# ChristophReich1996/Semantic_Pyramid_for_Image_Generation

Hardware: AMD Instinct MI355X
Metric: images/sec full G+D train step, 256x256, bs/GPU=20 (higher is better)
Workload: dtype bf16

## Files before the change

include/sempyr.h:

```cpp
#ifndef SEMPYR_H
#define SEMPYR_H
#include <stdint.h>

#ifdef __cplusplus
extern "C" {
#endif

#define SP_VERSION 1

typedef void* sp_stream_t;

enum sp_status { SP_OK = 0, SP_ERR_INVALID = -1, SP_ERR_LAUNCH = -2, SP_ERR_UNSUPPORTED = -3 };
enum sp_dtype { SP_F32 = 0, SP_BF16 = 1, SP_F8 = 2 ,
                SP_F16 = 3 ,
                SP_F8_F16 = 4  };
enum sp_act { SP_ACT_NONE = 0, SP_ACT_LRELU = 1, SP_ACT_RELU = 2, SP_ACT_TANH = 3 };

int sp_version(void);

enum { SP_TUNE_CONV_TALL = 0, SP_TUNE_IGEMM_DMA = 1, SP_TUNE_WGRAD_ROWS = 2, SP_TUNE_DETERMINISTIC = 3,
       SP_TUNE_SPLITK_TARGET = 4, SP_TUNE_SPLITK_MINSTEPS = 5, SP_TUNE_CONV1X1_DIRECT = 6, SP_TUNE_CONV_SHORT = 7,
       SP_TUNE_WGRAD9_BLOCKS = 8, SP_TUNE_WGRAD_BLOCKS = 9, SP_TUNE_WGRAD_MINSTEPS = 10, SP_TUNE_WGRAD_SMALL_M = 11,
       SP_TUNE_WGRAD_K1_TILE64 = 12, SP_TUNE_WGRAD_ROWS_THIN = 13, SP_TUNE_WGRAD_ROWS_BLOCKS = 14, SP_TUNE_WGRAD_ROWS_SLABS = 15,
       SP_TUNE_CONV_STAGGER = 16, SP_TUNE_CONV1X1_SPLITK = 17, SP_TUNE_WGRAD1X1 = 18, SP_TUNE_CONV_CIN8 = 19, SP_TUNE_CONV_THINCO = 20, SP_TUNE_CONV_PP = 21, SP_TUNE_CONV_PP_PRIO = 22, SP_TUNE_WGRAD_PP = 23, SP_TUNE_BN_ITERS = 24, SP_TUNE_IGEMM_TILE = 25, SP_TUNE_CONV_PPW = 26, SP_TUNE_LINEAR_KS = 27, SP_TUNE_CONV_PP_SPLIT = 28, SP_TUNE_COUNT = 29 };
int sp_set_tuning(int32_t key, int32_t value);
const char* sp_last_error_string(void);
const char* sp_last_route(void);

typedef struct sp_conv_params {
    const void* x;
    const void* w;
    const float* bias;
    void* y;
    const void* res1;
    const void* res2;
    const void* mask_src;
    float mask_neg_slope;
    int32_t n, h, w_, cin_p, cout, ldy, ksize, act, dtype;
    void* workspace;
    int64_t workspace_bytes;
    int32_t pool2;
    int32_t in_up2;
    const float* x_scale;
    const float* w_scale;
    void* y8;
    const float* y8_inv_scale;
    float* y8_amax;
    const float* img_scale;
    int32_t img_split;
    int32_t reserved_;
    int64_t split_pix_;
    const void* tail_w;
    const float* tail_bias;
    void* tail_y;
    int32_t tail_cout, tail_act, tail_ld, reserved2_;
    uint32_t* pool_idx;
    int32_t* split_sync;
} sp_conv_params;
#define SP_CONV_SPLIT_SYNC_BYTES 8192
int sp_conv2d_igemm(const sp_conv_params* p, sp_stream_t stream);
int sp_conv2d_workspace(int32_t n, int32_t h, int32_t w_, int32_t cin_p, int32_t cout, int32_t ksize, int32_t dtype,
                        int64_t* bytes_out);

int sp_conv2d_wgrad(const void* x, const void* dy, float* dw, int32_t n, int32_t h, int32_t w_,
                    int32_t cin_p, int32_t cout, int32_t ld_dy, int32_t ksize, int32_t dtype,
                    sp_stream_t stream);

int sp_conv2d_wgrad_fused(const void* x, const void* dy, float* dw, float* dbias, const void* w_packed, float* dot,
                          float* workspace, int64_t workspace_floats, int32_t n, int32_t h, int32_t w_, int32_t cin_p,
                          int32_t cout, int32_t ld_dy, int32_t ksize, int32_t dtype, sp_stream_t stream);
int sp_conv2d_wgrad_accum(const void* x, const void* dy, float* dw, float* dbias, float* workspace, int64_t workspace_floats,
                          int32_t n, int32_t h, int32_t w_, int32_t cin_p, int32_t cout, int32_t ld_dy, int32_t ksize,
                          int32_t dtype, sp_stream_t stream);
int sp_conv2d_wgrad_accum_pooled(const void* x, const void* dy, float* dw, float* dbias, float* workspace, int64_t workspace_floats,
                                 int32_t n, int32_t h, int32_t w_, int32_t cin_p, int32_t cout, int32_t ld_dy, int32_t ksize,
                                 int32_t dtype, sp_stream_t stream);
int sp_conv2d_wgrad_workspace(int32_t n, int32_t h, int32_t w_, int32_t cin_p, int32_t cout, int32_t ksize,
// ... 224 lines not shown
```

semantic_pyramid_for_image_generation_amd/_lib.py:

```python
from __future__ import annotations

import ctypes
import os
import re
from typing import Dict, List, Tuple

_HERE = os.path.dirname(os.path.abspath(__file__))
HEADER = os.path.join(os.path.dirname(_HERE), "include", "sempyr.h")
LIB_PATH = os.environ.get("SEMPYR_LIB") or os.path.join(_HERE, "libsempyr.so")

SP_F32, SP_BF16, SP_F8, SP_F16, SP_F8_F16 = 0, 1, 2, 3, 4
ACT_NONE, ACT_LRELU, ACT_RELU, ACT_TANH = 0, 1, 2, 3

TUNE_KEYS = {"SP_CONV_TALL": 0, "SP_IGEMM_DMA": 1, "SP_WGRAD_ROWS": 2, "SP_DETERMINISTIC": 3, "SP_SPLITK_TARGET": 4,
             "SP_SPLITK_MINSTEPS": 5, "SP_CONV1X1_DIRECT": 6, "SP_CONV_SHORT": 7, "SP_WGRAD9_BLOCKS": 8, "SP_WGRAD_BLOCKS": 9,
             "SP_WGRAD_MINSTEPS": 10, "SP_WGRAD_SMALL_M": 11, "SP_WGRAD_K1_TILE64": 12, "SP_WGRAD_ROWS_THIN": 13,
             "SP_WGRAD_ROWS_BLOCKS": 14, "SP_WGRAD_ROWS_SLABS": 15, "SP_CONV_STAGGER": 16, "SP_CONV1X1_SPLITK": 17, "SP_WGRAD1X1": 18, "SP_CONV_CIN8": 19, "SP_CONV_THINCO": 20,
             "SP_CONV_PP": 21, "SP_CONV_PP_PRIO": 22, "SP_WGRAD_PP": 23, "SP_BN_ITERS": 24, "SP_IGEMM_TILE": 25, "SP_CONV_PPW": 26, "SP_LINEAR_KS": 27, "SP_CONV_PP_SPLIT": 28}


SP_CONV_SPLIT_SYNC_BYTES = 8192


class SpConvParams(ctypes.Structure):
    _fields_ = [("x", ctypes.c_void_p), ("w", ctypes.c_void_p), ("bias", ctypes.c_void_p), ("y", ctypes.c_void_p),
                ("res1", ctypes.c_void_p), ("res2", ctypes.c_void_p), ("mask_src", ctypes.c_void_p),
                ("mask_neg_slope", ctypes.c_float),
                ("n", ctypes.c_int32), ("h", ctypes.c_int32), ("w_", ctypes.c_int32), ("cin_p", ctypes.c_int32),
                ("cout", ctypes.c_int32), ("ldy", ctypes.c_int32), ("ksize", ctypes.c_int32), ("act", ctypes.c_int32),
                ("dtype", ctypes.c_int32), ("workspace", ctypes.c_void_p), ("workspace_bytes", ctypes.c_int64),
                ("pool2", ctypes.c_int32), ("in_up2", ctypes.c_int32),
                ("x_scale", ctypes.c_void_p), ("w_scale", ctypes.c_void_p), ("y8", ctypes.c_void_p),
                ("y8_inv_scale", ctypes.c_void_p), ("y8_amax", ctypes.c_void_p),
                ("img_scale", ctypes.c_void_p), ("img_split", ctypes.c_int32), ("reserved_", ctypes.c_int32),
                ("split_pix_", ctypes.c_int64),
                ("tail_w", ctypes.c_void_p), ("tail_bias", ctypes.c_void_p), ("tail_y", ctypes.c_void_p),
                ("tail_cout", ctypes.c_int32), ("tail_act", ctypes.c_int32), ("tail_ld", ctypes.c_int32), ("reserved2_", ctypes.c_int32),
                ("pool_idx", ctypes.c_void_p), ("split_sync", ctypes.c_void_p)]


class SpConvGeneralParams(ctypes.Structure):
    _fields_ = [("struct_bytes", ctypes.c_int32), ("dtype", ctypes.c_int32),
                ("x", ctypes.c_void_p), ("w", ctypes.c_void_p), ("bias", ctypes.c_void_p), ("y", ctypes.c_void_p),
                ("n", ctypes.c_int32), ("h", ctypes.c_int32), ("w_", ctypes.c_int32), ("cin_p", ctypes.c_int32),
                ("ldx", ctypes.c_int32), ("cout", ctypes.c_int32), ("ldy", ctypes.c_int32), ("kh", ctypes.c_int32),
                ("kw", ctypes.c_int32), ("stride_h", ctypes.c_int32), ("stride_w", ctypes.c_int32), ("pad_h", ctypes.c_int32),
                ("pad_w", ctypes.c_int32), ("act", ctypes.c_int32)]

    def __init__(self, **kw):
        super().__init__(struct_bytes=ctypes.sizeof(SpConvGeneralParams), **kw)


class SpSnLayer(ctypes.Structure):
    _fields_ = [("w", ctypes.c_void_p), ("u", ctypes.c_void_p), ("v", ctypes.c_void_p),
                ("scratch_off", ctypes.c_int64), ("part_off", ctypes.c_int64), ("fwd_off", ctypes.c_int64),
                ("dgrad_off", ctypes.c_int64),
                ("rows", ctypes.c_int32), ("cols", ctypes.c_int32), ("cin", ctypes.c_int32), ("taps", ctypes.c_int32),
                ("cin_p", ctypes.c_int32), ("cout_p", ctypes.c_int32), ("kind", ctypes.c_int32),
                ("pack_block0", ctypes.c_int32)]


class SpSnBwdLayer(ctypes.Structure):
    _fields_ = [("w", ctypes.c_void_p), ("dw_off", ctypes.c_int64), ("dot_off", ctypes.c_int64),
                ("scratch_off", ctypes.c_int64), ("grad_off", ctypes.c_int64),
                ("rows", ctypes.c_int32), ("cols", ctypes.c_int32), ("cin", ctypes.c_int32), ("taps", ctypes.c_int32),
                ("cin_p", ctypes.c_int32), ("plain", ctypes.c_int32), ("db_off", ctypes.c_int32),
                ("bias_off", ctypes.c_int32)]


class SpRecLevel(ctypes.Structure):
    _fields_ = [("real", ctypes.c_void_p), ("fake", ctypes.c_void_p), ("mask", ctypes.c_void_p), ("dfake", ctypes.c_void_p),
# ... 60 lines not shown
```

semantic_pyramid_for_image_generation_amd/csrc/common.h:

```cpp
#pragma once
#include <hip/hip_runtime.h>
#include <stdint.h>
#include "../../include/sempyr.h"

typedef __attribute__((ext_vector_type(4))) float f32x4_t;
typedef __attribute__((ext_vector_type(4))) short s16x4_t;
typedef float sp_f32x2_t __attribute__((ext_vector_type(2)));

struct bf16 { uint16_t v; };
#ifdef SP_H16_FP16
typedef __attribute__((ext_vector_type(8))) _Float16 bf16x8_t;
typedef _Float16 sp_h16x2_t __attribute__((ext_vector_type(2)));
#define __builtin_amdgcn_mfma_f32_16x16x32_bf16 __builtin_amdgcn_mfma_f32_16x16x32_f16
#define SP_H16_ONE_PAIR 0x3C003C00u
__device__ __forceinline__ float bf16_bits_to_f32(uint32_t h) { return (float)__builtin_bit_cast(_Float16, (uint16_t)h); }
__device__ __forceinline__ uint32_t f32x2_to_bf16x2(float lo, float hi) {
    const sp_f32x2_t f = {lo, hi};
    return __builtin_bit_cast(uint32_t, __builtin_convertvector(f, sp_h16x2_t));
}
__device__ __forceinline__ float h16_lo_to_f32(uint32_t w) { return (float)__builtin_bit_cast(_Float16, (uint16_t)(w & 0xffffu)); }
__device__ __forceinline__ float h16_hi_to_f32(uint32_t w) { return (float)__builtin_bit_cast(_Float16, (uint16_t)(w >> 16)); }
#else
typedef __attribute__((ext_vector_type(8))) __bf16 bf16x8_t;
typedef __bf16 sp_bf16x2_t __attribute__((ext_vector_type(2)));
// ... 76 lines not shown
            asm("v_max_f32 %0, %1, %2" : "=v"(v[r]) : "v"(v[r]), "v"(s));
        }
    } else if (act == SP_ACT_RELU) {
#pragma unroll
        for (int r = 0; r < N; ++r) v[r] = fmaxf(v[r], 0.f);
    } else if (TANH_OK && act == SP_ACT_TANH) {
#pragma unroll
        for (int r = 0; r < N; ++r) v[r] = tanhf(v[r]);
    }
}

extern "C" void sp_set_error(const char* fmt, ...);
extern "C" void sp_note_route(const char* name);
#define SP_CHECK_ARG(cond, ...) do { if (!(cond)) { sp_set_error(__VA_ARGS__); return SP_ERR_INVALID; } } while (0)
#define SP_LAUNCH_CHECK() do { hipError_t e_ = hipGetLastError(); if (e_ != hipSuccess) { \
    sp_set_error("%s:%d HIP launch failed: %s", __FILE__, __LINE__, hipGetErrorString(e_)); return SP_ERR_LAUNCH; } } while (0)

static inline int sp_div_up(long a, long b) { return (int)((a + b - 1) / b); }

template <typename T, int V> struct VecIO;
template <> struct VecIO<float, 4> {
    static __device__ __forceinline__ void ld(const float* p, float (&o)[4]) { Elem<float>::ld4(p, o); }
    static __device__ __forceinline__ void st(float* p, const float (&o)[4]) { Elem<float>::st4(p, o); }
};
template <> struct VecIO<bf16, 4> {
    static __device__ __forceinline__ void ld(const bf16* p, float (&o)[4]) { Elem<bf16>::ld4(p, o); }
    static __device__ __forceinline__ void st(bf16* p, const float (&o)[4]) { Elem<bf16>::st4(p, o); }
};
template <> struct VecIO<bf16, 8> {
    static __device__ __forceinline__ void ld(const bf16* p, float (&o)[8]) {
        const uint4 v = *reinterpret_cast<const uint4*>(p);
        o[0] = bf16_bits_to_f32(v.x & 0xffffu); o[1] = bf16_bits_to_f32(v.x >> 16);
        o[2] = bf16_bits_to_f32(v.y & 0xffffu); o[3] = bf16_bits_to_f32(v.y >> 16);
        o[4] = bf16_bits_to_f32(v.z & 0xffffu); o[5] = bf16_bits_to_f32(v.z >> 16);
        o[6] = bf16_bits_to_f32(v.w & 0xffffu); o[7] = bf16_bits_to_f32(v.w >> 16);
    }
    static __device__ __forceinline__ void st(bf16* p, const float (&o)[8]) {
        uint4 v;
        v.x = f32x2_to_bf16x2(o[0], o[1]);
        v.y = f32x2_to_bf16x2(o[2], o[3]);
        v.z = f32x2_to_bf16x2(o[4], o[5]);
        v.w = f32x2_to_bf16x2(o[6], o[7]);
        *reinterpret_cast<uint4*>(p) = v;
    }
};

extern int* const sp_g_tune;
static inline int sp_tune(int key, int dflt) { return sp_g_tune[key] >= 0 ? sp_g_tune[key] : dflt; }
static inline bool sp_deterministic(int dtype) { return sp_g_tune[SP_TUNE_DETERMINISTIC] >= 0 ? sp_g_tune[SP_TUNE_DETERMINISTIC] != 0 : dtype == SP_F32; }
int sp_conv_pp_launch(const sp_conv_params& p, int th, hipStream_t s);
long sp_conv_pp_split_workspace(int n, int h, int w, int cin_p, int cout);
long sp_conv_pp_split_workspace_w16(int n, int h, int cin_p, int cout);
long sp_conv_pp_rounds100(long total, int cin_p, long workspace_bytes);
int sp_conv_ppw_launch(const sp_conv_params& p, hipStream_t s);
long sp_conv_ppw_split_workspace(int n, int h, int w, int cin_p, int cout);
long sp_conv_ppw_rounds100(long total, int cin_p, long workspace_bytes);
int sp_conv_ppw_covers(const sp_conv_params& p);
bool spq_push_reduce(const float* slabs, int nsplit, long n_dw, float* dw, const float* bias_slabs, int bias_ld, int cout, float* dbias);
int sp_wgrad_rows_launch(const void* x, const void* dy, float* dw, float* dbias, int n, int h, int w, int cin, int cout,
                         int ld_dy, float* ws, long ws_floats, int dy_up2, hipStream_t s);
long sp_wgrad_rows_workspace(int n, int h, int w, int cin, int cout);
int sp_wgrad_rows_launch_pair(const void* x, const void* dy, float* dw_a, float* dbias_a, float* dw_b, float* dbias_b, int n, int split,
                              int h, int w, int cin, int cout, int ld_dy, float* ws, long ws_floats, int dy_up2, hipStream_t s);
int sp_wgrad1x1_launch(const void* x, const void* dy, float* dw, float* dbias, int n, int h, int w, int cin, int cout, int ld_dy,
                       float* ws, long ws_floats, hipStream_t s);
long sp_wgrad1x1_workspace(int n, int h, int w, int cin, int cout, int ld_dy);
int sp_wgrad1x1_launch_pair(const void* x, const void* dy, float* dw_a, float* dbias_a, float* dw_b, float* dbias_b, int n, int split, int h, int w,
                            int cin, int cout, int ld_dy, float* ws, long ws_floats, hipStream_t s);
int sp_wgrad3x3_cin8_launch_pair(const void* x, const void* dy, float* dw_a, float* dbias_a, float* dw_b, float* dbias_b, int n, int split, int h,
                                 int w, int cout, int ld_dy, float* ws, long ws_floats, hipStream_t s);
int sp_wgrad3x3_cin8_launch(const void* x, const void* dy, float* dw, float* dbias, int n, int h, int w, int cout, int ld_dy, float* ws,
                            long ws_floats, hipStream_t s);
long sp_wgrad3x3_cin8_workspace(int n, int h, int w, int cout, int ld_dy);
```

semantic_pyramid_for_image_generation_amd/csrc/conv_igemm.hip:

```cpp
#include "conv_common.h"

namespace {

template <typename T, int WCO, int WPX, int FCO, int FPX>
__global__ __launch_bounds__(256) void conv_igemm_kernel(sp_conv_params p) {
    constexpr int CO_T = WCO * FCO * 16, PX_T = WPX * FPX * 16;
    constexpr int E = 16 / (int)sizeof(T);
    constexpr int KC = 8 * E;
    constexpr int W_CH = CO_T * 8, X_CH = PX_T * 8;
    constexpr int W_PER = (W_CH + 255) / 256, X_PER = (X_CH + 255) / 256;
    constexpr int STAGE = (CO_T + PX_T) * 128;
    extern __shared__ __attribute__((aligned(16))) char smem[];

    const int tid = threadIdx.x, lane = tid & 63, wave = tid >> 6;
    const int wco = wave / WPX, wpx = wave % WPX;
    const int H = p.h, W = p.w_, CIN = p.cin_p;
    const long M = (long)p.n * H * W;
    const long px0 = (long)blockIdx.x * PX_T;
    const int co0 = blockIdx.y * CO_T;
    const int taps = p.ksize * p.ksize;
    const int kchunks = (CIN + KC - 1) / KC;
    const int nk = taps * kchunks;
    const T* __restrict__ xg = reinterpret_cast<const T*>(p.x);
    const T* __restrict__ wg = reinterpret_cast<const T*>(p.w);
// ... 1322 lines not shown

template <int KC>
int launch_thinco(const sp_conv_params& p, hipStream_t s) {
    constexpr int LDS = TN_HH * TN_HW * (KC * 64 + 16);
    static bool attr_set = false;
    if (!attr_set) {
        hipError_t e = hipFuncSetAttribute(reinterpret_cast<const void*>(conv3x3_thinco_kernel<KC>), hipFuncAttributeMaxDynamicSharedMemorySize, LDS);
        if (e != hipSuccess) { sp_set_error("hipFuncSetAttribute(LDS=%d) failed: %s", LDS, hipGetErrorString(e)); return SP_ERR_LAUNCH; }
        attr_set = true;
    }
    const long blocks = (long)p.n * (p.h / TN_TH) * (p.w_ / TN_TW);
    sp_note_route("conv3x3_thinco");
    hipLaunchKernelGGL(conv3x3_thinco_kernel<KC>, dim3((unsigned)blocks), dim3(256), LDS, s, p);
    SP_LAUNCH_CHECK();
    return SP_OK;
}

template <typename T>
int dispatch(const sp_conv_params& p, hipStream_t s) {
    const long M = (long)p.n * p.h * p.w_;
    if (sizeof(T) == 2 && p.ksize == 3 && p.cout <= 4 && (p.cin_p == 32 || p.cin_p == 64) && !p.pool2 && !p.in_up2 && p.h % TN_TH == 0 &&
        p.w_ % TN_TW == 0 && sp_tune(SP_TUNE_CONV_THINCO, 1) && sp_tune(SP_TUNE_CONV_TALL, 1) <= 1)
        return p.cin_p == 64 ? launch_thinco<2>(p, s) : launch_thinco<1>(p, s);
    if (sizeof(T) == 2 && p.ksize == 3 && p.cin_p == 8 && p.cout % 16 == 0 && p.cout <= 64 && (p.ldy & 7) == 0 && !p.pool2 && !p.in_up2 &&
        p.h % C8_TH == 0 && p.w_ % C8_TW == 0 && sp_tune(SP_TUNE_CONV_CIN8, 1) && sp_tune(SP_TUNE_CONV_TALL, 1) <= 1)
        return launch_cin8(p, s);
    if (sizeof(T) == 2 && p.ksize == 1 && p.cin_p > 1024 && ((M + 31) / 32) * ((p.cout + 63) / 64) <= sp_tune(SP_TUNE_CONV1X1_SPLITK, 320))
        return launch_1x1_splitk(p, s);
    if (sizeof(T) == 2 && p.ksize == 1 && p.cin_p <= 1024) {
        const int ks = (p.cin_p + 31) / 32;
        const long blocks = ((M + 31) / 32) * ((p.cout + 63) / 64);
        if (ks >= 4 && ks <= 24 && blocks <= sp_tune(SP_TUNE_CONV1X1_SPLITK, 320)) return launch_1x1_splitk(p, s);
        if (sp_tune(SP_TUNE_CONV1X1_DIRECT, 1)) return launch_1x1_direct(p, s);
    }
    if (p.pool_idx != nullptr) {
        const long esz = p.dtype == SP_F32 ? 4 : 2;
        const bool fits30 = (long)p.n * p.h * p.w_ * p.cin_p * esz < (1L << 30) && (long)p.cout * 9 * p.cin_p * esz < (1L << 30);
        if (p.cout <= 64 && p.h % TL_TH != 0) return launch_halo<T, 64, 1, true>(p, s);
        if (!fits30) { sp_set_error("sp_conv2d_igemm: pool_idx needs operands below 1 GiB (n*h*w*cin_p, cout*9*cin_p)"); return SP_ERR_UNSUPPORTED; }
        if (sizeof(T) == 2 && sp_tune(SP_TUNE_CONV_PP, 1)) {
            const int rc = sp_conv_pp_launch(p, p.cout <= 64 ? 16 : 8, s);
            if (rc != 1) return rc;
        }
        return p.cout <= 64 ? launch_tall<T, 1, 16, true>(p, s) : launch_tall<T, 2, 8, true>(p, s);
    }
    const bool thin_big = p.cout <= 16 && p.cin_p >= 32 && M >= (1L << 18);
    if (p.ksize == 3 && (p.cout > 32 || thin_big) && p.h % HALO_TH == 0 && p.w_ % HALO_TW == 0) {
        const int tall_mode = sp_tune(SP_TUNE_CONV_TALL, 1);
        const long esz = p.dtype == SP_F32 ? 4 : 2;
        const bool fits30 = (long)p.n * p.h * p.w_ * p.cin_p * esz < (1L << 30) && (long)p.cout * 9 * p.cin_p * esz < (1L << 30);
        const bool tall_ok = tall_mode && fits30 && p.h % TL_TH == 0 && p.w_ % TL_TW == 0;
        if (p.cout <= 64) {
            if (tall_ok && sizeof(T) == 2 && p.cout > 16 && tall_mode <= 1 && sp_tune(SP_TUNE_CONV_PP, 1) && !(sp_tune(SP_TUNE_CONV_PP, 1) & 32)) {
                const int rc = sp_conv_pp_launch(p, 16, s);
                if (rc != 1) return rc;
            }
            if (tall_ok) return launch_tall<T, 1>(p, s);
            return launch_halo<T, 64, 1>(p, s);
        }
        const int pp_mode = sizeof(T) == 2 ? sp_tune(SP_TUNE_CONV_PP, 1) : 0;
        if (pp_mode && fits30 && tall_mode <= 1) {
            const long bt = (long)p.n * (p.h / TL_TH) * (p.w_ / TL_TW) * ((p.cout + 127) / 128);
            const long rt = (bt + 255) / 256, rh = (2 * bt + 255) / 256;
            int th = (tall_ok && 19 * rt < 10 * rh) ? 16 : 8;
            if (pp_mode == 8 || (pp_mode == 16 && tall_ok)) th = pp_mode;
            const int ppw_mode = sp_tune(SP_TUNE_CONV_PPW, 1);
            if (tall_ok && ppw_mode && pp_mode == 1 && sp_conv_ppw_covers(p)) {
                const int kch = (p.cin_p + 31) / 32;
                const long ratio = kch >= 12 ? 172 : kch >= 6 ? 185 : kch >= 3 ? 194 : 204;
                const long wsb = (p.workspace != nullptr && p.split_sync != nullptr) ? p.workspace_bytes : 0;
                const long rh100 = sp_conv_pp_rounds100(2 * bt, p.cin_p, wsb);
                const long rt100 = ppw_mode == 3 ? sp_conv_ppw_rounds100(bt, p.cin_p, wsb) : 100 * rt;
                if (ppw_mode == 2 || ratio * rt100 < 100 * rh100) {
                    const int rc = sp_conv_ppw_launch(p, s);
                    if (rc != 1) return rc;
                }
                th = 8;
            }
            if (!(pp_mode == 1 && th == 16)) {
                const int rc = sp_conv_pp_launch(p, th, s);
                if (rc != 1) return rc;
            }
        }
        if (tall_ok) {
            const long bt = (long)p.n * (p.h / TL_TH) * (p.w_ / TL_TW) * ((p.cout + 127) / 128);
            const long rt = (bt + 255) / 256, rh = (2 * bt + 255) / 256;
            if (tall_mode == 2 || 19 * rt < 10 * rh) return launch_tall<T, 2>(p, s);
        }
        const int short_env = sp_tune(SP_TUNE_CONV_SHORT, 1);
        if (fits30 && (tall_mode == 3 || (tall_mode == 1 && short_env))) return launch_tall<T, 2, 8>(p, s);
        return launch_halo<T, 128, 3>(p, s);
    }
    if (sizeof(T) == 2 && p.ksize == 3 && p.w_ == 16 && p.cout > 64) {
        const int ppm = sp_tune(SP_TUNE_CONV_PP, 1);
        if (ppm == 1 || ppm == 3) {
            const int rc = sp_conv_pp_launch(p, 1616, s);
            if (rc != 1) return rc;
        }
    }
    const int dma_mode = sp_tune(SP_TUNE_IGEMM_DMA, 1);
    const long esz_ = p.dtype == SP_F32 ? 4 : 2;
    const bool dma_fits = M * p.cin_p * esz_ < (1L << 30) && (long)p.cout * p.ksize * p.ksize * p.cin_p * esz_ < (1L << 30);
    if (p.cout > 16 && dma_fits && (dma_mode == 2 || (dma_mode == 1 && p.ksize == 3 && M <= 8192))) {
        if (p.cout <= 32) return launch_dma<T, 1, 4, 2, 4>(p, s);
        if (p.cout <= 64) return launch_dma<T, 1, 4, 4, 4>(p, s);
        if (M <= 8192) {
            switch (igemm_small_tile(M, p.cout, p.cin_p, p.ksize, p.dtype)) {
// ... 103 lines not shown
```

semantic_pyramid_for_image_generation_amd/csrc/conv_pp.hip:

```cpp
#include "conv_common.h"

namespace {

constexpr int PP_TW_WIDE = 32;
constexpr int PP_NUM_CU = 256;
constexpr int PP_BIAS_MAX = 1024;

constexpr int PP_SK_MAX_PARTS = 4;
constexpr int PP_SK_SLAB_FLOATS = 8 * 64 * 64;

struct PPSplit { int parts, tail_items, grid; };
inline PPSplit pp_split_plan(int total, int kchunks, long workspace_bytes) {
    PPSplit r{0, 0, total < PP_NUM_CU ? total : PP_NUM_CU};
    const int mode = sp_tune(SP_TUNE_CONV_PP_SPLIT, 1);
    if (!mode || total <= 0 || (total < PP_NUM_CU && mode == 2)) return r;
    const int R = total % PP_NUM_CU;
    if (R == 0) return r;
    int pmax = PP_NUM_CU / R;
    if (pmax > PP_SK_MAX_PARTS) pmax = PP_SK_MAX_PARTS;
    int P = 1;
    long best = 37L * kchunks;
    const long handover = total >= 2 * PP_NUM_CU ? 40 : 60;
    for (int q = 2; q <= pmax && kchunks / q >= 2; ++q) {
        const long c = 37L * ((kchunks + q - 1) / q) + handover * (q - 1);
// ... 650 lines not shown
    constexpr int LDS_BYTES = TAIL ? G::LDS_TAIL : G::LDS;
    static_assert(LDS_BYTES <= 163840, "LDS budget");
    static bool attr_set = false;
    auto kern = conv3x3_pp_kernel<T, WCO, PRIO, TIMING, DMA_IN_L, FAST, FW, TAIL, IDX>;
    if (!attr_set) {
        hipError_t e = hipFuncSetAttribute(reinterpret_cast<const void*>(kern), hipFuncAttributeMaxDynamicSharedMemorySize, LDS_BYTES);
        if (e != hipSuccess) { sp_set_error("hipFuncSetAttribute(LDS=%d) failed: %s", LDS_BYTES, hipGetErrorString(e)); return SP_ERR_LAUNCH; }
        attr_set = true;
    }
    const int cotiles = (p.cout + G::CO_T - 1) / G::CO_T;
    const int total = p.n * (p.h / TH) * (p.w_ / G::TW) * cotiles;
    PPSplit sk = pp_split_plan(total, (p.cin_p + G::KC - 1) / G::KC,
                               (!G::F8 && !TIMING && !TAIL && p.workspace != nullptr && p.split_sync != nullptr) ? p.workspace_bytes : 0);
    const int grid = sk.grid;
    sp_note_route(G::F8 ? "conv3x3_pp<f8,2>" : FW == 1 ? "conv3x3_pp<16bit,2,FAST,w16>" : WCO == 2 ? (FAST ? "conv3x3_pp<16bit,2,FAST>" : "conv3x3_pp<16bit,2>")
                                                                                  : (FAST ? "conv3x3_pp<16bit,1,FAST>" : "conv3x3_pp<16bit,1>"));
        hipLaunchKernelGGL(kern, dim3((unsigned)grid), dim3(512), LDS_BYTES, s, p, cotiles, total, prio, sk.parts | (sp_tune(SP_TUNE_CONV_PP_SPLIT, 1) == 3 ? 256 : 0));
    SP_LAUNCH_CHECK();
    return SP_OK;
}

}

long sp_conv_pp_split_workspace(int n, int h, int w, int cin_p, int cout) {
    if (h % 8 != 0 || w % PP_TW_WIDE != 0 || cout <= 16) return 0;
    const int kchunks = (cin_p + 31) / 32;
    long need = 0;
    auto plan = [&](long total) {
        if (total >= (1L << 30)) return;
        const PPSplit sk = pp_split_plan((int)total, kchunks, 1L << 40);
        const long b = (long)sk.tail_items * (sk.parts > 1 ? sk.parts : 0) * PP_SK_SLAB_FLOATS * 4;
        if (b > need) need = b;
    };
    if (cout <= 64) { if (h % 16 == 0) plan((long)n * (h / 16) * (w / PP_TW_WIDE)); }
    else plan((long)n * (h / 8) * (w / PP_TW_WIDE) * ((cout + 127) / 128));
    return need;
}

long sp_conv_pp_split_workspace_w16(int n, int h, int cin_p, int cout) {
    if (h % 16 != 0 || cout <= 64 || (long)n * (h / 16) * ((cout + 127) / 128) < 64) return 0;
    const PPSplit sk = pp_split_plan(n * (h / 16) * ((cout + 127) / 128), (cin_p + 31) / 32, 1L << 40);
    return (long)sk.tail_items * (sk.parts > 1 ? sk.parts : 0) * PP_SK_SLAB_FLOATS * 4;
}

long sp_conv_pp_rounds100(long total, int cin_p, long workspace_bytes) {
    const int kchunks = (cin_p + 31) / 32;
    if (total < (1L << 30)) {
        const PPSplit sk = pp_split_plan((int)total, kchunks, workspace_bytes);
        if (sk.parts > 1 && total >= PP_NUM_CU) return 100 * (total / PP_NUM_CU) + 100 / sk.parts + 162 * (sk.parts - 1) / kchunks + 1;
    }
    return 100 * ((total + PP_NUM_CU - 1) / PP_NUM_CU);
}

int sp_conv_pp_launch(const sp_conv_params& p, int th, hipStream_t s) {
    if (p.dtype == SP_F8) {
        if (p.ksize != 3 || p.cout <= 64 || p.h % 8 != 0 || p.w_ % PP_TW_WIDE != 0 || (long)p.n * p.h * p.w_ * p.cin_p >= (1L << 30) ||
            (long)p.cout * 9 * p.cin_p >= (1L << 30) || (p.cout + 127) / 128 * 128 > PP_BIAS_MAX) return 1;
        return launch_pp<f8, 2, 1>(p, 1, s);
    }
    if (p.dtype != SP_BF16 || p.ksize != 3) return 1;
    const long esz = 2;
    if (th == 1616) {
        if (p.w_ != 16 || p.h % 16 != 0 || (long)p.n * (p.h / 16) * ((p.cout + 127) / 128) < 64 || p.pool2 != 0 || (p.cout & 15) != 0 || (p.ldy & 7) != 0 || p.act == SP_ACT_TANH) return 1;
        if ((long)p.n * p.h * p.w_ * p.cin_p * esz >= (1L << 30) || (long)p.cout * 9 * p.cin_p * esz >= (1L << 30)) return 1;
        return launch_pp<bf16, 2, 1, false, true, true, 1>(p, 1, s);
    }
    if (p.h % th != 0 || p.w_ % PP_TW_WIDE != 0) return 1;
    if ((long)p.n * p.h * p.w_ * p.cin_p * esz >= (1L << 30) || (long)p.cout * 9 * p.cin_p * esz >= (1L << 30)) return 1;
    const int prio = sp_tune(SP_TUNE_CONV_PP_PRIO, 1);
    const bool fast = !(prio & 16) && p.pool2 == 0 && (p.cout & 15) == 0 && (p.ldy & 7) == 0 && p.act != SP_ACT_TANH;
    if (p.tail_w != nullptr) {
        if (!(th == 16 && p.cout == 64 && fast)) return 1;
        return launch_pp<bf16, 1, 1, false, true, true, 2, true>(p, prio, s);
    }
    if (p.pool_idx != nullptr) {
        if (p.pool2 != 2) return 1;
        if (th == 16 && p.cout <= 64) return launch_pp<bf16, 1, 1, false, true, false, 2, false, true>(p, prio, s);
        if (th == 8 && p.cout > 64) return launch_pp<bf16, 2, 1, false, true, false, 2, false, true>(p, prio, s);
        return 1;
    }
    if (th == 16 && p.cout <= 64) {
        if ((prio & 4) && fast && p.workspace != nullptr && p.workspace_bytes >= 256L * 8 * 16 * 4)
            return launch_pp<bf16, 1, 1, true, true, true>(p, prio, s);
        return fast ? launch_pp<bf16, 1, 1, false, true, true>(p, prio, s) : launch_pp<bf16, 1, 1>(p, prio, s);
    }
    if (th != 8 || p.cout <= 64) return 1;
    if ((prio & 4) && p.workspace != nullptr && p.workspace_bytes >= 256L * 8 * 16 * 4)
        return fast ? launch_pp<bf16, 2, 1, true, true, true>(p, prio, s) : launch_pp<bf16, 2, 1, true>(p, prio, s);
    return fast ? launch_pp<bf16, 2, 1, false, true, true>(p, prio, s) : launch_pp<bf16, 2, 1>(p, prio, s);
}
```

Before: 1390.

## Add persistent pipelined 3x3 conv kernel specialised for cout up to 64

Adds a persistent 3x3 bf16 convolution kernel for layers with 16 < cout <= 64. It uses buffer-to-LDS DMA with double-buffered halo tiles, a four-slot weight ring and MFMA compute. The epilogue stores of the previous tile overlap the next tile's main loop. It runs before the existing pp path for thin-output layers and falls back when split-K would be chosen or when unsupported fusions are present. The goal is better CU use and latency hiding on low-cout convolutions, at the cost of a large new kernel that carries its own correctness risk.

```diff
diff --git a/include/sempyr.h b/include/sempyr.h
--- a/include/sempyr.h
+++ b/include/sempyr.h
@@ -22,7 +22,7 @@
        SP_TUNE_SPLITK_TARGET = 4, SP_TUNE_SPLITK_MINSTEPS = 5, SP_TUNE_CONV1X1_DIRECT = 6, SP_TUNE_CONV_SHORT = 7,
        SP_TUNE_WGRAD9_BLOCKS = 8, SP_TUNE_WGRAD_BLOCKS = 9, SP_TUNE_WGRAD_MINSTEPS = 10, SP_TUNE_WGRAD_SMALL_M = 11,
        SP_TUNE_WGRAD_K1_TILE64 = 12, SP_TUNE_WGRAD_ROWS_THIN = 13, SP_TUNE_WGRAD_ROWS_BLOCKS = 14, SP_TUNE_WGRAD_ROWS_SLABS = 15,
-       SP_TUNE_CONV_STAGGER = 16, SP_TUNE_CONV1X1_SPLITK = 17, SP_TUNE_WGRAD1X1 = 18, SP_TUNE_CONV_CIN8 = 19, SP_TUNE_CONV_THINCO = 20, SP_TUNE_CONV_PP = 21, SP_TUNE_CONV_PP_PRIO = 22, SP_TUNE_WGRAD_PP = 23, SP_TUNE_BN_ITERS = 24, SP_TUNE_IGEMM_TILE = 25, SP_TUNE_CONV_PPW = 26, SP_TUNE_LINEAR_KS = 27, SP_TUNE_CONV_PP_SPLIT = 28, SP_TUNE_COUNT = 29 };
+       SP_TUNE_CONV_STAGGER = 16, SP_TUNE_CONV1X1_SPLITK = 17, SP_TUNE_WGRAD1X1 = 18, SP_TUNE_CONV_CIN8 = 19, SP_TUNE_CONV_THINCO = 20, SP_TUNE_CONV_PP = 21, SP_TUNE_CONV_PP_PRIO = 22, SP_TUNE_WGRAD_PP = 23, SP_TUNE_BN_ITERS = 24, SP_TUNE_IGEMM_TILE = 25, SP_TUNE_CONV_PPW = 26, SP_TUNE_LINEAR_KS = 27, SP_TUNE_CONV_PP_SPLIT = 28, SP_TUNE_CONV_PP64 = 29, SP_TUNE_COUNT = 30 };
 int sp_set_tuning(int32_t key, int32_t value);
 const char* sp_last_error_string(void);
 const char* sp_last_route(void);
diff --git a/semantic_pyramid_for_image_generation_amd/_lib.py b/semantic_pyramid_for_image_generation_amd/_lib.py
--- a/semantic_pyramid_for_image_generation_amd/_lib.py
+++ b/semantic_pyramid_for_image_generation_amd/_lib.py
@@ -16,7 +16,7 @@
              "SP_SPLITK_MINSTEPS": 5, "SP_CONV1X1_DIRECT": 6, "SP_CONV_SHORT": 7, "SP_WGRAD9_BLOCKS": 8, "SP_WGRAD_BLOCKS": 9,
              "SP_WGRAD_MINSTEPS": 10, "SP_WGRAD_SMALL_M": 11, "SP_WGRAD_K1_TILE64": 12, "SP_WGRAD_ROWS_THIN": 13,
              "SP_WGRAD_ROWS_BLOCKS": 14, "SP_WGRAD_ROWS_SLABS": 15, "SP_CONV_STAGGER": 16, "SP_CONV1X1_SPLITK": 17, "SP_WGRAD1X1": 18, "SP_CONV_CIN8": 19, "SP_CONV_THINCO": 20,
-             "SP_CONV_PP": 21, "SP_CONV_PP_PRIO": 22, "SP_WGRAD_PP": 23, "SP_BN_ITERS": 24, "SP_IGEMM_TILE": 25, "SP_CONV_PPW": 26, "SP_LINEAR_KS": 27, "SP_CONV_PP_SPLIT": 28}
+             "SP_CONV_PP": 21, "SP_CONV_PP_PRIO": 22, "SP_WGRAD_PP": 23, "SP_BN_ITERS": 24, "SP_IGEMM_TILE": 25, "SP_CONV_PPW": 26, "SP_LINEAR_KS": 27, "SP_CONV_PP_SPLIT": 28, "SP_CONV_PP64": 29}
 
 
 SP_CONV_SPLIT_SYNC_BYTES = 8192
diff --git a/semantic_pyramid_for_image_generation_amd/csrc/common.h b/semantic_pyramid_for_image_generation_amd/csrc/common.h
--- a/semantic_pyramid_for_image_generation_amd/csrc/common.h
+++ b/semantic_pyramid_for_image_generation_amd/csrc/common.h
@@ -152,6 +152,8 @@
 long sp_conv_pp_split_workspace(int n, int h, int w, int cin_p, int cout);
 long sp_conv_pp_split_workspace_w16(int n, int h, int cin_p, int cout);
 long sp_conv_pp_rounds100(long total, int cin_p, long workspace_bytes);
+int sp_conv_pp_split_parts(int total, int cin_p, long workspace_bytes);
+int sp_conv_pp64_launch(const sp_conv_params& p, hipStream_t s);
 int sp_conv_ppw_launch(const sp_conv_params& p, hipStream_t s);
 long sp_conv_ppw_split_workspace(int n, int h, int w, int cin_p, int cout);
 long sp_conv_ppw_rounds100(long total, int cin_p, long workspace_bytes);
diff --git a/semantic_pyramid_for_image_generation_amd/csrc/conv_igemm.hip b/semantic_pyramid_for_image_generation_amd/csrc/conv_igemm.hip
--- a/semantic_pyramid_for_image_generation_amd/csrc/conv_igemm.hip
+++ b/semantic_pyramid_for_image_generation_amd/csrc/conv_igemm.hip
@@ -1398,7 +1398,9 @@
         const bool tall_ok = tall_mode && fits30 && p.h % TL_TH == 0 && p.w_ % TL_TW == 0;
         if (p.cout <= 64) {
             if (tall_ok && sizeof(T) == 2 && p.cout > 16 && tall_mode <= 1 && sp_tune(SP_TUNE_CONV_PP, 1) && !(sp_tune(SP_TUNE_CONV_PP, 1) & 32)) {
-                const int rc = sp_conv_pp_launch(p, 16, s);
+                int rc = sp_conv_pp64_launch(p, s);
+                if (rc != 1) return rc;
+                rc = sp_conv_pp_launch(p, 16, s);
                 if (rc != 1) return rc;
             }
             if (tall_ok) return launch_tall<T, 1>(p, s);
diff --git a/semantic_pyramid_for_image_generation_amd/csrc/conv_pp.hip b/semantic_pyramid_for_image_generation_amd/csrc/conv_pp.hip
--- a/semantic_pyramid_for_image_generation_amd/csrc/conv_pp.hip
+++ b/semantic_pyramid_for_image_generation_amd/csrc/conv_pp.hip
@@ -726,6 +726,10 @@
     return 100 * ((total + PP_NUM_CU - 1) / PP_NUM_CU);
 }
 
+int sp_conv_pp_split_parts(int total, int cin_p, long workspace_bytes) {
+    return pp_split_plan(total, (cin_p + 31) / 32, workspace_bytes).parts;
+}
+
 int sp_conv_pp_launch(const sp_conv_params& p, int th, hipStream_t s) {
     if (p.dtype == SP_F8) {
         if (p.ksize != 3 || p.cout <= 64 || p.h % 8 != 0 || p.w_ % PP_TW_WIDE != 0 || (long)p.n * p.h * p.w_ * p.cin_p >= (1L << 30) ||
diff --git a/semantic_pyramid_for_image_generation_amd/csrc/conv_pp64.hip b/semantic_pyramid_for_image_generation_amd/csrc/conv_pp64.hip
--- /dev/null
+++ b/semantic_pyramid_for_image_generation_amd/csrc/conv_pp64.hip
@@ -0,0 +1,399 @@
+#include "conv_common.h"
+
+namespace {
+
+constexpr int P64_TW = 32, P64_TH = 16, P64_CO = 64;
+constexpr int P64_KC = 32;
+constexpr int P64_HR = P64_TH + 2, P64_HP = 40;
+constexpr int P64_HALO_INSTR = (P64_HR * P64_HP * 64 + 1023) / 1024;
+constexpr int P64_HALO_BUF = P64_HALO_INSTR * 1024;
+constexpr int P64_HPW = (P64_HALO_INSTR + 7) / 8;
+constexpr int P64_HPS0 = (P64_HPW + 1) / 2, P64_HPS1 = P64_HPW - P64_HPS0;
+constexpr int P64_W_BYTES = 3 * P64_CO * 64, P64_W_INSTR = P64_W_BYTES / 1024, P64_W_PER = (P64_W_INSTR + 7) / 8;
+constexpr int P64_NWS = 4;
+constexpr int P64_BIAS_MAX = 1024;
+constexpr int P64_OFF_W = 2 * P64_HALO_BUF, P64_OFF_BIAS = P64_OFF_W + P64_NWS * P64_W_BYTES, P64_OFF_DUMMY = P64_OFF_BIAS + P64_BIAS_MAX * 4;
+constexpr int P64_LDS = P64_OFF_DUMMY + 1024;
+constexpr int P64_NUM_CU = 256;
+constexpr int RW = 2, FW = 2, NB = RW + 2, NFR = RW * FW;
+
+template <typename T, int PRIO>
+__global__ __launch_bounds__(512) void conv3x3_pp64_kernel(sp_conv_params p, int total, int prio) {
+    constexpr int E = 16 / (int)sizeof(T), KC = P64_KC, TH = P64_TH, HP = P64_HP;
+    constexpr int HALO_INSTR = P64_HALO_INSTR, HALO_BUF = P64_HALO_BUF, HPW = P64_HPW, W_BYTES = P64_W_BYTES, W_PER = P64_W_PER, W_INSTR = P64_W_INSTR;
+    static_assert(E == 8, "16-bit operands");
+    extern __shared__ __attribute__((aligned(16))) char smem[];
+    const int tid = threadIdx.x, lane = tid & 63;
+    const int wave = __builtin_amdgcn_readfirstlane(tid >> 6);
+    const int wpx = wave;
+    const bool half_b = wave >= 4;
+    const int H = p.h, W = p.w_, CIN = p.cin_p;
+    const int tiles_x = W / P64_TW, tiles_y = H / TH;
+    const int kchunks = (CIN + KC - 1) / KC;
+    const T* __restrict__ wg = reinterpret_cast<const T*>(p.w);
+    const unsigned lds_base = (unsigned)(uintptr_t)((__attribute__((address_space(3))) char*)smem);
+    const int GR = gridDim.x;
+    int bid = blockIdx.x;
+    if ((GR & 7) == 0) bid = (bid & 7) * (GR >> 3) + (bid >> 3);
+    const int my_items = (total - bid + GR - 1) / GR;
+    const int nchunks = my_items * kchunks;
+    if (nchunks <= 0) return;
+
+    {
+        float* bias_l = reinterpret_cast<float*>(smem + P64_OFF_BIAS);
+        for (int i = tid; i < P64_CO; i += 512) bias_l[i] = (p.bias != nullptr && i < p.cout) ? p.bias[i] : 0.f;
+    }
+
+    constexpr unsigned OOB = 0x80000000u, OOB_C = 0x40000000u;
+    const int up = p.in_up2 ? 1 : 0;
+    const int HS = H >> up, WS = W >> up;
+    auto uniform_ptr = [](const void* q) {
+        const unsigned long long v = (unsigned long long)(uintptr_t)q;
+        const unsigned lo = __builtin_amdgcn_readfirstlane((unsigned)v), hi = __builtin_amdgcn_readfirstlane((unsigned)(v >> 32));
+        return (void*)(uintptr_t)(((unsigned long long)hi << 32) | lo);
+    };
+    const __amdgpu_buffer_rsrc_t x_rsrc = __builtin_amdgcn_make_buffer_rsrc(uniform_ptr(p.x), 0,
+        __builtin_amdgcn_readfirstlane(p.n * HS * WS * CIN * (int)sizeof(T)), 0x00020000);
+    const __amdgpu_buffer_rsrc_t w_rsrc = __builtin_amdgcn_make_buffer_rsrc(uniform_ptr(wg), 0,
+        __builtin_amdgcn_readfirstlane(p.cout * 9 * CIN * (int)sizeof(T)), 0x00020000);
+    const int ls = ((lane & 3) ^ ((lane >> 3) & 3)) * E;
+    unsigned h_off[HPW], w_off[W_PER];
+    struct Coords { int tx_i, ty_i, n; };
+    Coords cur, nxt;
+    int s_tx, s_ty, s_n;
+    {
+        int t = bid;
+        cur.tx_i = t % tiles_x; t /= tiles_x;
+        cur.ty_i = t % tiles_y; cur.n = t / tiles_y;
+        t = GR;
+        s_tx = t % tiles_x; t /= tiles_x;
+        s_ty = t % tiles_y; s_n = t / tiles_y;
+    }
+    auto advance = [&](const Coords& c) {
+        Coords r;
+        r.tx_i = c.tx_i + s_tx; int cy = r.tx_i >= tiles_x ? 1 : 0; r.tx_i -= cy ? tiles_x : 0;
+        r.ty_i = c.ty_i + s_ty + cy; cy = r.ty_i >= tiles_y ? 1 : 0; r.ty_i -= cy ? tiles_y : 0;
+        r.n = c.n + s_n + cy;
+        return r;
+    };
+    nxt = advance(cur);
+    auto set_halo_desc = [&](const Coords& c) {
+        const int n = c.n, ty0 = c.ty_i * TH, tx0 = c.tx_i * P64_TW;
+        int l4 = lane >> 2;
+        asm volatile("" : "+v"(l4));
+#pragma unroll
+        for (int i = 0; i < HPW; ++i) {
+            const int hp = (i * 8 + wave) * 16 + l4;
+            const int hy = hp / HP, hx = hp - hy * HP;
+            const int yy = ty0 - 1 + hy, xx = tx0 - 1 + hx;
+            const bool ok = hx < P64_TW + 2 && hy < P64_HR && (unsigned)yy < (unsigned)H && (unsigned)xx < (unsigned)W;
+            h_off[i] = ok ? (unsigned)((((n * HS + (yy >> up)) * WS + (xx >> up)) * CIN + ls) * (int)sizeof(T)) : OOB;
+        }
+    };
+    auto w_ls = [&](int i) { return ((lane & 3) ^ (((lane >> 3) & 1) | (((wave * W_PER + i) & 1) << 1))) * E; };
+    auto set_w_desc = [&]() {
+        int l4 = lane >> 2;
+        asm volatile("" : "+v"(l4));
+#pragma unroll
+        for (int i = 0; i < W_PER; ++i) {
+            const int row = (wave * W_PER + i) * 16 + l4;
+            const int ts = row / P64_CO, co = row % P64_CO;
+            w_off[i] = (wave * W_PER + i < W_INSTR && co < p.cout) ? (unsigned)(((co * 9 + ts * 3) * CIN + w_ls(i)) * (int)sizeof(T)) : OOB;
+        }
+    };
+    auto dma = [&](__amdgpu_buffer_rsrc_t rsrc, unsigned dst, unsigned voff) {
+        __builtin_amdgcn_raw_ptr_buffer_load_lds(rsrc, (__attribute__((address_space(3))) void*)(smem + dst), 16, (int)voff, 0, 0, 0);
+    };
+    auto issue_halo_piece = [&](int i, bool valid, int c0, int slot) {
+        const unsigned add = c0 + ls < CIN ? (unsigned)(c0 * (int)sizeof(T)) : OOB_C;
+        const int q = i * 8 + wave;
+        const unsigned m = (valid && q < HALO_INSTR) ? 0xffffffffu : 0u;
+        dma(x_rsrc, ((unsigned)(slot * HALO_BUF + q * 1024) & m) | ((unsigned)P64_OFF_DUMMY & ~m), ((h_off[i] + add) & m) | (OOB & ~m));
+    };
+    auto issue_w_piece = [&](int i, bool valid, int c0, int ds, int slot) {
+        const unsigned base = (unsigned)((ds * CIN + c0) * (int)sizeof(T));
+        const unsigned add = c0 + w_ls(i) < CIN ? base : OOB_C;
+        const unsigned m = (valid && wave * W_PER + i < W_INSTR) ? 0xffffffffu : 0u;
+        dma(w_rsrc, ((unsigned)(P64_OFF_W + slot * W_BYTES + (wave * W_PER + i) * 1024) & m) | ((unsigned)P64_OFF_DUMMY & ~m),
+            ((w_off[i] + add) & m) | (OOB & ~m));
+    };
+
+    const int frow = lane & 15, fslot = lane >> 4;
+    const unsigned a_addr = lds_base + P64_OFF_W + ((frow >> 2) * 16 + (frow & 3)) * 64 +
+                            ((fslot ^ (((frow >> 1) & 1) | (((frow >> 2) & 1) << 1))) << 4);
+    unsigned b_addr[3];
+#pragma unroll
+    for (int ds = 0; ds < 3; ++ds)
+        b_addr[ds] = lds_base + ((RW * wpx) * HP + frow + ds) * 64 + ((fslot ^ (((frow + ds) >> 1) & 3)) << 4);
+    const int co_b = (lane >> 4) * 16;
+    const unsigned bias_addr = lds_base + P64_OFF_BIAS + co_b * 4;
+
+    const bool bias_in_acc = p.bias != nullptr && !up && p.img_scale == nullptr;
+    f32x4_t acc[4][NFR];
+    uint4 b4[4];
+    auto bias_fetch = [&](bool live) {
+#pragma unroll
+        for (int i = 0; i < 4; ++i) b4[i] = make_uint4(0, 0, 0, 0);
+        if (bias_in_acc && live) {
+            lds_rd128<0>(b4[0], bias_addr); lds_rd128<16>(b4[1], bias_addr); lds_rd128<32>(b4[2], bias_addr); lds_rd128<48>(b4[3], bias_addr);
+            wait_lgkm<0>();
+        }
+    };
+
+    set_halo_desc(cur);
+    set_w_desc();
+#pragma unroll
+    for (int i = 0; i < HPW; ++i) issue_halo_piece(i, true, 0, 0);
+#pragma unroll
+    for (int ds = 0; ds < 3; ++ds)
+#pragma unroll
+        for (int i = 0; i < W_PER; ++i) issue_w_piece(i, true, 0, ds, ds);
+    wait_vmcnt<2 * W_PER>();
+    asm volatile("s_waitcnt lgkmcnt(0)" ::: "memory");
+    __builtin_amdgcn_s_barrier();
+    __builtin_amdgcn_sched_barrier(0);
+    bias_fetch(true);
+    auto acc_from_bias = [&]() {
+#pragma unroll
+        for (int i = 0; i < 4; ++i)
+#pragma unroll
+            for (int j = 0; j < NFR; ++j) acc[i][j] = __builtin_bit_cast(f32x4_t, b4[i]);
+    };
+    acc_from_bias();
+    if (half_b) __builtin_amdgcn_s_barrier();
+    if ((prio & 2) && half_b) __builtin_amdgcn_s_setprio(1);
+
+    f32x4_t pend[4][NFR];
+    long poff0 = 0;
+    bool parked = false;
+    const bool wide = co_b < p.cout;
+    const T* const op_src[2] = {reinterpret_cast<const T*>(p.mask_src), reinterpret_cast<const T*>(p.res1)};
+    uint4 opd[2][2];
+    auto operands_landed = [&]() {
+#pragma unroll
+        for (int o = 0; o < 2; ++o)
+#pragma unroll
+            for (int h = 0; h < 2; ++h) asm volatile("" :: "v"(opd[o][h].x), "v"(opd[o][h].y), "v"(opd[o][h].z), "v"(opd[o][h].w));
+    };
+    auto foff = [&](int j) { return poff0 + ((long)(j / FW) * W + (j % FW) * 16) * p.ldy; };
+    auto load_operands = [&](auto jc) {
+        constexpr int j = decltype(jc)::value;
+        if (wide) {
+#pragma unroll
+            for (int o = 0; o < 2; ++o)
+                if (op_src[o] != nullptr) {
+                    const T* q = op_src[o] + foff(j);
+                    opd[o][0] = *reinterpret_cast<const uint4*>(q);
+                    opd[o][1] = *reinterpret_cast<const uint4*>(q + 8);
+                }
+        }
+    };
+    auto piece = [&](auto jc) {
+        constexpr int j = decltype(jc)::value;
+        operands_landed();
+        if (wide) {
+            f32x4_t v[4];
+#pragma unroll
+            for (int i = 0; i < 4; ++i) v[i] = pend[i][j];
+            auto with_operand = [&](int o, auto&& apply) {
+#pragma unroll
+                for (int k = 0; k < 8; ++k) {
+                    const uint4& u = opd[o][k >> 2];
+                    const uint32_t w = (k & 3) == 0 ? u.x : (k & 3) == 1 ? u.y : (k & 3) == 2 ? u.z : u.w;
+                    v[k >> 1][2 * (k & 1)] = apply(v[k >> 1][2 * (k & 1)], h16_lo_to_f32(w));
+                    v[k >> 1][2 * (k & 1) + 1] = apply(v[k >> 1][2 * (k & 1) + 1], h16_hi_to_f32(w));
+                }
+            };
+            if (p.mask_src != nullptr) {
+                const float slope = p.mask_neg_slope;
+                with_operand(0, [&](float a, float t) { return a * (t > 0.f ? 1.f : slope); });
+            }
+            if (p.res1 != nullptr) with_operand(1, [](float a, float t) { return a + t; });
+            if (p.act == SP_ACT_LRELU) {
+#pragma unroll
+                for (int i = 0; i < 4; ++i) {
+                    const f32x4_t sv = v[i] * 0.2f;
+#pragma unroll
+                    for (int r = 0; r < 4; ++r) {
+                        const float av = v[i][r], s1 = sv[r];
+                        float mv;
+                        asm("v_max_f32 %0, %1, %2" : "=v"(mv) : "v"(av), "v"(s1));
+                        v[i][r] = mv;
+                    }
+                }
+            } else if (p.act == SP_ACT_RELU) {
+#pragma unroll
+                for (int i = 0; i < 4; ++i)
+#pragma unroll
+                    for (int r = 0; r < 4; ++r) v[i][r] = fmaxf(v[i][r], 0.f);
+            }
+            if (p.y != nullptr) {
+                unsigned w8[8];
+#pragma unroll
+                for (int k = 0; k < 8; ++k) w8[k] = f32x2_to_bf16x2(v[k >> 1][2 * (k & 1)], v[k >> 1][2 * (k & 1) + 1]);
+                T* q = reinterpret_cast<T*>(p.y) + foff(j);
+                *reinterpret_cast<uint4*>(q) = make_uint4(w8[0], w8[1], w8[2], w8[3]);
+                *reinterpret_cast<uint4*>(q + 8) = make_uint4(w8[4], w8[5], w8[6], w8[7]);
+            }
+        }
+        if constexpr (j + 1 < NFR) load_operands(std::integral_constant<int, j + 1>{});
+        else parked = false;
+    };
+
+    int g4 = 0;
+    int kc = 0;
+    for (int gc = 0; gc < nchunks; ++gc) {
+        const bool more_chunks = gc + 1 < nchunks;
+        const bool item_ends = kc + 1 == kchunks;
+        const unsigned hb = (unsigned)((gc & 1) * HALO_BUF);
+        const int c0_next = item_ends ? 0 : (kc + 1) * KC;
+        auto stage = [&](auto sc) {
+            constexpr int st = decltype(sc)::value;
+            constexpr int NREAD = 12 + FW * NB;
+            constexpr int TAP_STRIDE = P64_CO * 64;
+            constexpr int NH = st == 0 ? P64_HPS0 : st == 1 ? P64_HPS1 : 0, H0 = st == 0 ? 0 : P64_HPS0;
+            constexpr int NPIECE = NH + W_PER;
+            const unsigned ab = a_addr + (unsigned)(g4 * W_BYTES);
+            const unsigned bb = b_addr[st] + hb;
+            uint4 a[3][4], bf[NB][FW];
+            const int ws = (g4 + 3) & 3;
+            auto dma_piece = [&](auto kc_) {
+                constexpr int k = decltype(kc_)::value;
+                if constexpr (k < NH) issue_halo_piece(H0 + k, more_chunks, c0_next, (gc + 1) & 1);
+                else if constexpr (k < NPIECE) issue_w_piece(k - NH, more_chunks, c0_next, st, ws);
+            };
+            if constexpr (st == 0) {
+                if (item_ends && more_chunks) set_halo_desc(nxt);
+            }
+            static_for<((NREAD + 3) / 4 > NPIECE ? (NREAD + 3) / 4 : NPIECE)>([&](auto qc) {
+                constexpr int q0 = decltype(qc)::value * 4;
+                static_for<4>([&](auto rc) {
+                    constexpr int r = q0 + decltype(rc)::value;
+                    if constexpr (r < 12) {
+                        lds_rd128<(r / 4) * TAP_STRIDE + (r % 4) * 256>(a[r / 4][r % 4], ab);
+                    } else if constexpr (r < NREAD) {
+                        constexpr int h = (r - 12) / FW, hh = (r - 12) % FW;
+                        lds_rd128<h * (HP * 64) + hh * 1024>(bf[h][hh], bb);
+                    }
+                });
+                dma_piece(qc);
+            });
+            wait_vmcnt<st == 0 ? 2 * W_PER + P64_HPS0 : st == 1 ? 2 * W_PER + P64_HPS0 + P64_HPS1 : 2 * W_PER>();
+            wait_lgkm<0>();
+            __builtin_amdgcn_s_barrier();
+            __builtin_amdgcn_sched_barrier(0);
+            if constexpr (PRIO) __builtin_amdgcn_s_setprio(1);
+            static_for<NB * 3>([&](auto gi) {
+                constexpr int h = decltype(gi)::value / 3, dr = decltype(gi)::value % 3, rr = h - dr;
+                if constexpr (rr >= 0 && rr < RW) {
+#pragma unroll
+                    for (int i = 0; i < 4; ++i)
+#pragma unroll
+                        for (int hh = 0; hh < FW; ++hh) Mma<T>::run(a[dr][i], bf[h][hh], acc[i][rr * FW + hh]);
+                }
+            });
+            if constexpr (PRIO) __builtin_amdgcn_s_setprio(0);
+            __builtin_amdgcn_sched_barrier(0);
+            if (parked) {
+                if (kc == 0) piece(std::integral_constant<int, st>{});
+                else if constexpr (st == 0) { if (kc == 1) piece(std::integral_constant<int, 3>{}); }
+            }
+            __builtin_amdgcn_sched_barrier(0);
+            if (!(st == 2 && item_ends && half_b)) __builtin_amdgcn_s_barrier();
+            __builtin_amdgcn_sched_barrier(0);
+            g4 = (g4 + 1) & 3;
+        };
+        stage(std::integral_constant<int, 0>{});
+        stage(std::integral_constant<int, 1>{});
+        stage(std::integral_constant<int, 2>{});
+        if (item_ends) {
+            const int n = cur.n, ty0 = cur.ty_i * TH, tx0 = cur.tx_i * P64_TW;
+            if (up) {
+#pragma unroll
+                for (int i = 0; i < 4; ++i)
+#pragma unroll
+                    for (int j = 0; j < NFR; ++j) acc[i][j] *= 0.25f;
+            }
+            if (p.img_scale != nullptr) {
+                const float sc = p.img_scale[n >= p.img_split ? 1 : 0];
+#pragma unroll
+                for (int i = 0; i < 4; ++i)
+#pragma unroll
+                    for (int j = 0; j < NFR; ++j) acc[i][j] *= sc;
+            }
+            if (!bias_in_acc && p.bias != nullptr) {
+                uint4 t4[4];
+                lds_rd128<0>(t4[0], bias_addr); lds_rd128<16>(t4[1], bias_addr); lds_rd128<32>(t4[2], bias_addr); lds_rd128<48>(t4[3], bias_addr);
+                wait_lgkm<0>();
+                if (wide) {
+#pragma unroll
+                    for (int c = 0; c < 16; ++c) {
+                        const uint4& u = t4[c >> 2];
+                        const float t = __uint_as_float((c & 3) == 0 ? u.x : (c & 3) == 1 ? u.y : (c & 3) == 2 ? u.z : u.w);
+#pragma unroll
+                        for (int jj = 0; jj < NFR; ++jj) acc[c >> 2][jj][c & 3] += t;
+                    }
+                }
+            }
+#pragma unroll
+            for (int i = 0; i < 4; ++i)
+#pragma unroll
+                for (int j = 0; j < NFR; ++j) pend[i][j] = acc[i][j];
+            poff0 = (((long)n * H + ty0 + RW * wpx) * W + tx0 + (lane & 15)) * p.ldy + co_b;
+            parked = true;
+            operands_landed();
+            load_operands(std::integral_constant<int, 0>{});
+            cur = nxt;
+            nxt = advance(nxt);
+            kc = 0;
+            bias_fetch(more_chunks);
+            acc_from_bias();
+            if (half_b) { __builtin_amdgcn_s_barrier(); __builtin_amdgcn_sched_barrier(0); }
+        } else {
+            ++kc;
+        }
+    }
+    if (!half_b) __builtin_amdgcn_s_barrier();
+    if (parked) {
+        piece(std::integral_constant<int, 0>{});
+        piece(std::integral_constant<int, 1>{});
+        piece(std::integral_constant<int, 2>{});
+        piece(std::integral_constant<int, 3>{});
+    }
+}
+
+template <typename T>
+int launch_pp64(const sp_conv_params& p, int prio, hipStream_t s) {
+    static bool attr_set = false;
+    auto kern = conv3x3_pp64_kernel<T, 1>;
+    static_assert(P64_LDS <= 163840, "LDS budget");
+    if (!attr_set) {
+        hipError_t e = hipFuncSetAttribute(reinterpret_cast<const void*>(kern), hipFuncAttributeMaxDynamicSharedMemorySize, P64_LDS);
+        if (e != hipSuccess) { sp_set_error("hipFuncSetAttribute(LDS=%d) failed: %s", P64_LDS, hipGetErrorString(e)); return SP_ERR_LAUNCH; }
+        attr_set = true;
+    }
+    const int total = p.n * (p.h / P64_TH) * (p.w_ / P64_TW);
+    const int grid = total < P64_NUM_CU ? total : P64_NUM_CU;
+    sp_note_route("conv3x3_pp64<16bit,FAST>");
+    hipLaunchKernelGGL(kern, dim3((unsigned)grid), dim3(512), P64_LDS, s, p, total, prio);
+    SP_LAUNCH_CHECK();
+    return SP_OK;
+}
+
+}
+
+int sp_conv_pp64_launch(const sp_conv_params& p, hipStream_t s) {
+    if (!sp_tune(SP_TUNE_CONV_PP64, 1)) return 1;
+    if (p.dtype != SP_BF16 || p.ksize != 3 || p.cout <= 16 || p.cout > 64 || p.cin_p <= P64_KC) return 1;
+    if (p.h % P64_TH != 0 || p.w_ % P64_TW != 0) return 1;
+    const long esz = 2;
+    if ((long)p.n * p.h * p.w_ * p.cin_p * esz >= (1L << 30) || (long)p.cout * 9 * p.cin_p * esz >= (1L << 30)) return 1;
+    const int prio = sp_tune(SP_TUNE_CONV_PP_PRIO, 1);
+    const bool fast = !(prio & 16) && !(prio & 4) && p.pool2 == 0 && (p.cout & 15) == 0 && (p.ldy & 7) == 0 && p.act != SP_ACT_TANH;
+    if (!fast || p.tail_w != nullptr || p.pool_idx != nullptr || p.res2 != nullptr) return 1;
+    const long total = (long)p.n * (p.h / P64_TH) * (p.w_ / P64_TW);
+    if (total >= (1L << 30)) return 1;
+    const long wsb = (p.workspace != nullptr && p.split_sync != nullptr) ? p.workspace_bytes : 0;
+    if (sp_conv_pp_split_parts((int)total, p.cin_p, wsb) > 1) return 1;
+    return launch_pp64<bf16>(p, prio, s);
+}
```

Result: no change. 1389 (median of 2 runs) (-0.1%).
